# Liz490/multimodal_alzheimer

Hardware: AMD Instinct MI355X
Metric: volumes/sec fwd+bwd, 3D-ResNet-10 @128^3 bf16, 1/2/4/8 MI355X; % HBM roofline (higher is better)
Workload: dtype bf16; 1 GPU; BASELINE config 2: Anat_CNN ResNet-10 MRI-only, 1x128^3, batch 8/GPU, weighted CE, Adam, fwd+bwd+step; global_batch=8, parallelism=dp1, step_launch=hip graph replay

## Files before the change

### include/mmad.h

```cpp
#ifndef MMAD_H
#define MMAD_H

#include <stdint.h>

#ifdef __cplusplus
extern "C" {
#endif

enum { MMAD_OK = 0, MMAD_EBADSHAPE = 1001, MMAD_EBADDTYPE = 1002, MMAD_ENULL = 1003,
       MMAD_EUNSUPPORTED = 1004, MMAD_EHIP = 2000 };

enum { MMAD_F32 = 0, MMAD_BF16 = 1, MMAD_F64 = 2, MMAD_F16 = 3, MMAD_BITS = 4 };

typedef struct mmad_conv_desc {
  int32_t n;
  int32_t ci, di, hi, wi;
  int32_t co, do_, ho, wo;
  int32_t kd, kh, kw;
  int32_t sd, sh, sw;
  int32_t pd, ph, pw;
  int32_t dd, dh, dw;
} mmad_conv_desc;

int mmad_abi_version(void);
// ... 131 lines not shown
                       const void* relu_out, const void* y, const float* mean,
                       const float* invstd, float* parts, void* stream);
int mmad_bn_bwd_finalize(int c, int64_t count, int nparts, const float* parts,
                         const float* gamma, const float* invstd, int training,
                         float* dgamma, float* dbeta, float* coef, void* stream);
int mmad_bn_bwd_apply(int dtype, int64_t m, int c, const void* g, const void* g2,
                      const void* relu_out, const void* y, const float* mean,
                      const float* invstd, const float* coef, void* dy, void* gmask_out,
                      void* stream);
int mmad_bn_bwd_reduce2(int dtype, int64_t m, int c, const void* g, const void* g2,
                        int64_t g_rows, const void* relu_out, const void* y, const float* mean,
                        const float* invstd, const void* y2,
                        const float* mean2, const float* invstd2, float* parts, float* parts2,
                        void* stream);
int mmad_bn_bwd_finalize2(int c, int64_t count, int nparts, const float* parts,
                          const float* gamma, const float* invstd, int training, float* dgamma,
                          float* dbeta, float* coef, const float* parts2, const float* gamma2,
                          const float* invstd2, int training2, float* dgamma2, float* dbeta2,
                          float* coef2, void* stream);
int mmad_bn_bwd_apply2(int dtype, int64_t m, int c, const void* g, const void* g2,
                       int64_t g_rows, const void* relu_out, const void* y, const float* mean, const float* invstd, const float* coef,
                       void* dy, const void* y2, const float* mean2, const float* invstd2,
                       const float* coef2, void* dy2, void* stream);
int mmad_bn_relu_bwd_reduce(int dtype, int64_t m, int c, const void* g, const void* y,
                            const float* mean, const float* invstd, const float* scale,
                            const float* shift, float* parts, void* stream);
int mmad_bn_relu_bwd_apply(int dtype, int64_t m, int c, const void* g, const void* y,
                           const float* mean, const float* invstd, const float* scale,
                           const float* shift, const float* coef, void* dy, void* stream);
int mmad_relu_fwd(int dtype, int64_t n, const void* x, void* y, void* stream);
int mmad_relu_bwd(int dtype, int64_t n, const void* g, const void* out, void* dx, void* stream);
int mmad_add(int dtype, int64_t n, const void* a, const void* b, void* out, void* stream);

int mmad_colsum_ws(int dtype, int64_t m, int c, const void* y, float* parts, float* out,
                   void* stream);
int mmad_maxpool3d_fwd(int dtype, int n, int c, int di, int hi, int wi, int do_, int ho,
                       int wo, int k, int s, int p, const void* x, void* y,
                       uint8_t* argmax, void* stream);
int mmad_maxpool3d_bwd(int dtype, int n, int c, int di, int hi, int wi, int do_, int ho,
                       int wo, int k, int s, int p, const void* dy, const uint8_t* argmax,
                       void* dx, void* stream);
int mmad_bnpool_fwd(int dtype, int n, int c, int di, int hi, int wi, int do_, int ho, int wo,
                    int k, int s, int p, const void* y, const float* scale, const float* shift,
                    void* out, uint8_t* argmax, void* ymax, void* stream);
int mmad_bnpool_bwd_reduce(int dtype, int64_t m, int c, const void* g, const void* g2,
                           void* gsum, const uint8_t* argmax, const void* ymax,
// ... 129 lines not shown
```

### multimodal_alzheimer_amd/_lib.py

```python
import ctypes as C
import os

import torch

_PKG = os.path.dirname(os.path.abspath(__file__))
LIB_PATH = os.environ.get("MMAD_LIB_PATH") or os.path.join(_PKG, "libmmad_hip.so")

F32, BF16, F64 = 0, 1, 2
F16, BITS = 3, 4
EUNSUPPORTED = 1004
EHIP = 2000
_HIP_OOM = 2

_vp, _i32, _i64, _f32, _f64, _u64 = C.c_void_p, C.c_int, C.c_int64, C.c_float, C.c_double, C.c_uint64


class ConvDesc(C.Structure):
    _fields_ = [(n, C.c_int32) for n in (
        "n", "ci", "di", "hi", "wi", "co", "do_", "ho", "wo", "kd", "kh", "kw",
        "sd", "sh", "sw", "pd", "ph", "pw", "dd", "dh", "dw")]


class PackJob(C.Structure):
    _fields_ = ([("w", C.c_void_p), ("w_packed", C.c_void_p)] +
# ... 79 lines not shown
    "mmad_wgrad_reduce_batch": (_i32, [_i32, C.POINTER(WgradJob), _vp]),
    "mmad_stem_raw_ok": (_i32, [_P, _i32, _i32]),
    "mmad_conv3d_fwd_raw": (_i32, [_P, _i32, _vp, _i32, _vp, _vp, _vp, _vp, _vp]),
    "mmad_conv3d_wgrad_raw": (_i32, [_P, _i32, _vp, _i32, _vp, _vp, _vp, _vp, _vp, _vp]),
    "mmad_stem_dgrad_ok": (_i32, [_P, _i32, _i32]),
    "mmad_stem_dgrad_ws_bytes": (_i64, [_P]),
    "mmad_conv3d_dgrad_raw": (_i32, [_P, _i32, _vp, _vp, _i32, _vp, _vp, _vp]),
    "mmad_bn_stats_parts": (_i64, [_i64, _i32]),
    "mmad_bn_stats": (_i32, [_i32, _i64, _i32, _vp, _vp, _vp]),
    "mmad_bn_parts_fold": (_i32, [_i32, _i32, _vp, _i32, _vp, _vp]),
    "mmad_bn_finalize": (_i32, [_i32, _i64, _i32, _vp, _vp, _vp, _vp, _vp, _f32, _f32, _i32,
                                _vp, _vp, _vp, _vp, _vp, _vp]),
    "mmad_bn_finalize2": (_i32, [_i32, _i64, C.POINTER(BnFin), C.POINTER(BnFin), _vp]),
    "mmad_scale_shift_act": (_i32, [_i32, _i64, _i32, _vp, _vp, _vp, _vp, _vp, _vp, _i32, _vp,
                                    _vp]),
    "mmad_bn_bwd_parts": (_i64, [_i64, _i32]),
    "mmad_bn_bwd_reduce": (_i32, [_i32, _i64, _i32] + [_vp] * 8),
    "mmad_bn_bwd_finalize": (_i32, [_i32, _i64, _i32, _vp, _vp, _vp, _i32, _vp, _vp, _vp, _vp]),
    "mmad_bn_bwd_apply": (_i32, [_i32, _i64, _i32] + [_vp] * 10),
    "mmad_bn_bwd_reduce2": (_i32, [_i32, _i64, _i32, _vp, _vp, _i64] + [_vp] * 10),
    "mmad_bn_bwd_finalize2": (_i32, [_i32, _i64, _i32, _vp, _vp, _vp, _i32, _vp, _vp, _vp,
                                     _vp, _vp, _vp, _i32, _vp, _vp, _vp, _vp]),
    "mmad_bn_bwd_apply2": (_i32, [_i32, _i64, _i32, _vp, _vp, _i64] + [_vp] * 12),
    "mmad_relu_fwd": (_i32, [_i32, _i64, _vp, _vp, _vp]),
    "mmad_relu_bwd": (_i32, [_i32, _i64, _vp, _vp, _vp, _vp]),
    "mmad_colsum_ws": (_i32, [_i32, _i64, _i32, _vp, _vp, _vp, _vp]),
    "mmad_add": (_i32, [_i32, _i64, _vp, _vp, _vp, _vp]),
    "mmad_maxpool3d_fwd": (_i32, [_i32] * 12 + [_vp, _vp, _vp, _vp]),
    "mmad_maxpool3d_bwd": (_i32, [_i32] * 12 + [_vp, _vp, _vp, _vp]),
    "mmad_bnpool_fwd": (_i32, [_i32] * 12 + [_vp] * 7),
    "mmad_bnpool_bwd_reduce": (_i32, [_i32, _i64, _i32] + [_vp] * 9),
    "mmad_bnpool_bwd_apply": (_i32, [_i32] * 12 + [_vp] * 8),
    "mmad_gap_fwd": (_i32, [_i32, _i32, _i64, _i32, _vp, _vp, _vp]),
    "mmad_gap_fwd_ws_elems": (_i64, [_i32, _i64, _i32]),
    "mmad_conv3d_fwd_ex": (_i32, [_P, _i32, _vp, _vp, _vp, _vp, _i32, _vp, _vp, _vp]),
    "mmad_conv_pack_weight_scaled": (_i32, [_P, _i32, _vp, _vp, _vp, _i32, _vp]),
    "mmad_bn_fold": (_i32, [_i32, _vp, _vp, _vp, _vp, _f32, _vp, _vp, _vp, _vp]),
    "mmad_norm_ws_bytes": (_i64, [_i32, _i64]),
    "mmad_mri_minmax_norm": (_i32, [_i32, _i64, _vp, _vp, _f64, _vp, _vp, _vp, _vp]),
    "mmad_mri_zscore_norm": (_i32, [_i32, _i64, _vp, _vp, _vp, _vp, _vp]),
    "mmad_affine_norm": (_i32, [_i64, _vp, _f64, _f64, _vp, _vp]),
    "mmad_gap_fwd_ws": (_i32, [_i32, _i32, _i64, _i32, _vp, _vp, _vp, _vp]),
    "mmad_gap_bwd": (_i32, [_i32, _i32, _i64, _i32, _vp, _vp, _vp]),
    "mmad_gap_bwd_compact": (_i32, [_i32, _i32, _i64, _i32, _vp, _vp, _vp]),
    "mmad_gap_parts": (_i32, [_i32, _i64, _i32]),
    "mmad_gap_partial": (_i32, [_i32, _i32, _i64, _i32, _vp, _vp, _vp]),
# ... 118 lines not shown
```

### multimodal_alzheimer_amd/csrc/bn.hip

```cpp
#include "common.h"

constexpr int COLSUM_ROWS = 4;

namespace {

struct PartPlan {
  int64_t rpp;
  int nparts;
};
PartPlan part_plan(int64_t M) {
  int n = (int)std::min<int64_t>(1024, std::max<int64_t>(1, cdiv(M, 64)));
  const int64_t rpp = cdiv(M, n);
  return {rpp, (int)cdiv(M, rpp)};
}

#ifndef BN_FOLD_PROBE
#define BN_FOLD_PROBE 0
#endif
#if BN_FOLD_PROBE
__device__ int g_fold_cnt[4096];
__device__ float g_fold_sink[4096];
#endif

template <typename T, int MODE, int V, bool DUAL = false, bool G2 = false, bool GB = false>
__global__ __launch_bounds__(256) void colsum_kernel(int64_t M, int C, int64_t rpp,
                                                     const T* __restrict__ y,
                                                     const T* __restrict__ g,
                                                     const T* __restrict__ relu_out,
                                                     const float* __restrict__ mean,
                                                     const float* __restrict__ invstd,
                                                     float* __restrict__ parts,
                                                     const uint8_t* __restrict__ act,
                                                     const float* __restrict__ msc,
                                                     const float* __restrict__ msh,
                                                     const T* __restrict__ y2 = nullptr,
                                                     const float* __restrict__ mean2 = nullptr,
                                                     const float* __restrict__ invstd2 = nullptr,
                                                     float* __restrict__ parts2 = nullptr,
                                                     const T* __restrict__ g2 = nullptr,
                                                     T* __restrict__ gsum = nullptr,
                                                     uint32_t gS = 0) {
  static_assert(!DUAL || MODE == 1, "dual partial sums: BN backward with a relu_out mask");
  static_assert(!GB || (DUAL && V == Chunk<T>::N), "broadcast g: the pair kernel, 16-byte rows");
  __shared__ float red[DUAL ? 3 : 2][2048];
  const int tid = threadIdx.x;
  const int CC = C / (int)gridDim.y;
  const int cb = (int)blockIdx.y * CC;
  const int lpr = CC / V;
  const int rpar = 256 / lpr;
  const int cl = tid % lpr, rl = tid / lpr;
  const int64_t r0 = (int64_t)blockIdx.x * rpp;
  const int64_t r1 = min(M, r0 + rpp);
  float s[V], q[V], q2[V];
#pragma unroll
  for (int e = 0; e < V; ++e) { s[e] = 0.f; q[e] = 0.f; q2[e] = 0.f; }
  if (rl < rpar) {
    float mu[V], is[V], sc[V], sh[V], mu2[V], is2[V];
    if (MODE == 1 || MODE == 3 || MODE == 4) {
#pragma unroll
      for (int e = 0; e < V; ++e) { mu[e] = mean[cb + cl * V + e]; is[e] = invstd[cb + cl * V + e]; }
    }
    if constexpr (DUAL) {
#pragma unroll
      for (int e = 0; e < V; ++e) {
        mu2[e] = mean2[cb + cl * V + e];
        is2[e] = invstd2[cb + cl * V + e];
      }
    }
    if (MODE == 4) {
#pragma unroll
      for (int e = 0; e < V; ++e) { sc[e] = msc[cb + cl * V + e]; sh[e] = msh[cb + cl * V + e]; }
    }
    auto accum = [&](int64_t i, float* yv, float* gv, const float* ov, const float* y2v) {
      if (MODE == 1 || MODE == 3 || MODE == 4) {
        if (MODE == 4) {
#pragma unroll
          for (int e = 0; e < V; ++e) gv[e] = bn_affine(yv[e], sc[e], sh[e]) > 0.f ? gv[e] : 0.f;
        } else if (MODE == 3) {
#pragma unroll
          for (int e = 0; e < V; ++e) gv[e] = (act[i + e] & 0x80) ? gv[e] : 0.f;
        } else if (relu_out != nullptr) {
#pragma unroll
          for (int e = 0; e < V; ++e) gv[e] = ov[e] > 0.f ? gv[e] : 0.f;
        }
#pragma unroll
        for (int e = 0; e < V; ++e) {
          s[e] += gv[e];
          q[e] += gv[e] * ((yv[e] - mu[e]) * is[e]);
        }
        if constexpr (DUAL) {
#pragma unroll
          for (int e = 0; e < V; ++e) q2[e] += gv[e] * ((y2v[e] - mu2[e]) * is2[e]);
        }
      } else {
#pragma unroll
        for (int e = 0; e < V; ++e) {
          s[e] += yv[e];
          if (MODE == 0) q[e] += yv[e] * yv[e];
        }
      }
    };
    constexpr bool NEED_G = MODE == 1 || MODE == 3 || MODE == 4;
    int64_t r = r0 + rl;
    if constexpr (V == Chunk<T>::N) {
      constexpr int U = COLSUM_ROWS;
      for (; r + (U - 1) * rpar < r1; r += U * rpar) {
        u32x4 yr[U], gr[U], orr[U], y2r[U], g2r[U];
#pragma unroll
        for (int u = 0; u < U; ++u) {
          const int64_t i = (r + u * rpar) * C + cb + cl * V;
          yr[u] = *reinterpret_cast<const u32x4*>(y + i);
          if constexpr (GB)
            gr[u] = *reinterpret_cast<const u32x4*>(
                g + (int64_t)((uint32_t)(r + u * rpar) / gS) * C + cb + cl * V);
          else if (NEED_G)
            gr[u] = *reinterpret_cast<const u32x4*>(g + i);
          if (NEED_G && G2) g2r[u] = *reinterpret_cast<const u32x4*>(g2 + i);
          if (MODE == 1 && relu_out != nullptr)
            orr[u] = *reinterpret_cast<const u32x4*>(relu_out + i);
          if constexpr (DUAL) y2r[u] = *reinterpret_cast<const u32x4*>(y2 + i);
        }
#pragma unroll
        for (int u = 0; u < U; ++u) {
          const int64_t i = (r + u * rpar) * C + cb + cl * V;
          float yv[V], gv[V], ov[V], y2v[V];
          Chunk<T>::load(reinterpret_cast<const T*>(&yr[u]), yv);
          if (NEED_G) Chunk<T>::load(reinterpret_cast<const T*>(&gr[u]), gv);
          if constexpr (NEED_G && G2) {
            float hv[V];
            Chunk<T>::load(reinterpret_cast<const T*>(&g2r[u]), hv);
#pragma unroll
            for (int e = 0; e < V; ++e) gv[e] = as_stored<T>(gv[e] + hv[e]);
            if constexpr (MODE == 3) Chunk<T>::store(gsum + i, gv);
          }
          if (MODE == 1 && relu_out != nullptr)
            Chunk<T>::load(reinterpret_cast<const T*>(&orr[u]), ov);
          if constexpr (DUAL) Chunk<T>::load(reinterpret_cast<const T*>(&y2r[u]), y2v);
          accum(i, yv, gv, ov, y2v);
        }
      }
    }
    for (; r < r1; r += rpar) {
      const int64_t i = r * C + cb + cl * V;
      float yv[V], gv[V], ov[V], y2v[V];
      if constexpr (V == Chunk<T>::N) Chunk<T>::load(y + i, yv);
      else for (int e = 0; e < V; ++e) yv[e] = Elt<T>::ld(y, i + e);
      if (NEED_G) {
        if constexpr (GB) Chunk<T>::load(g + (int64_t)((uint32_t)r / gS) * C + cb + cl * V, gv);
        else if constexpr (V == Chunk<T>::N) Chunk<T>::load(g + i, gv);
        else for (int e = 0; e < V; ++e) gv[e] = Elt<T>::ld(g, i + e);
        if constexpr (G2) {
          float hv[V];
          if constexpr (V == Chunk<T>::N) Chunk<T>::load(g2 + i, hv);
          else for (int e = 0; e < V; ++e) hv[e] = Elt<T>::ld(g2, i + e);
#pragma unroll
          for (int e = 0; e < V; ++e) gv[e] = as_stored<T>(gv[e] + hv[e]);
          if constexpr (MODE == 3) {
            if constexpr (V == Chunk<T>::N) Chunk<T>::store(gsum + i, gv);
            else for (int e = 0; e < V; ++e) Elt<T>::st(gsum, i + e, gv[e]);
          }
        }
        if (MODE == 1 && relu_out != nullptr) {
          if constexpr (V == Chunk<T>::N) Chunk<T>::load(relu_out + i, ov);
          else for (int e = 0; e < V; ++e) ov[e] = Elt<T>::ld(relu_out, i + e);
        }
      }
      if constexpr (DUAL) {
        if constexpr (V == Chunk<T>::N) Chunk<T>::load(y2 + i, y2v);
        else for (int e = 0; e < V; ++e) y2v[e] = Elt<T>::ld(y2, i + e);
      }
      accum(i, yv, gv, ov, y2v);
    }
#pragma unroll
    for (int e = 0; e < V; ++e) {
      red[0][rl * CC + cl * V + e] = s[e];
      red[1][rl * CC + cl * V + e] = q[e];
      if constexpr (DUAL) red[DUAL ? 2 : 0][rl * CC + cl * V + e] = q2[e];
    }
  }
  __syncthreads();
  for (int c = tid; c < CC; c += 256) {
    float ss = 0.f, qq = 0.f, q2q = 0.f;
    for (int k = 0; k < rpar; ++k) {
      ss += red[0][k * CC + c];
      qq += red[1][k * CC + c];
// ... 320 lines not shown
      v[e] = relu ? fmaxf(o, 0.f) : o;
    }
  };
  int64_t q = t0;
  for (; q + stride < nchunks; q += 2 * stride) {
    float v0[N], v1[N], r0[N], r1[N];
    Chunk<T>::load(y + q * N, v0);
    Chunk<T>::load(y + (q + stride) * N, v1);
    if (RES) {
      Chunk<T>::load(res + q * N, r0);
      Chunk<T>::load(res + (q + stride) * N, r1);
    }
    apply(v0, r0);
    apply(v1, r1);
    Chunk<T>::store(out + q * N, v0);
    Chunk<T>::store(out + (q + stride) * N, v1);
  }
  if (q < nchunks) {
    float v0[N], r0[N];
    Chunk<T>::load(y + q * N, v0);
    if (RES) Chunk<T>::load(res + q * N, r0);
    apply(v0, r0);
    Chunk<T>::store(out + q * N, v0);
  }
}

template <typename T>
__global__ void scale_shift_act_scalar_kernel(int64_t M, int C, const T* __restrict__ y,
                                              const float* __restrict__ scale,
                                              const float* __restrict__ shift,
                                              const T* __restrict__ res,
                                              const float* __restrict__ rscale,
                                              const float* __restrict__ rshift, int relu,
                                              T* __restrict__ out) {
  const int64_t n = M * C;
  for (int64_t i = blockIdx.x * (int64_t)blockDim.x + threadIdx.x; i < n;
       i += (int64_t)gridDim.x * blockDim.x) {
    const int c = (int)(i % C);
    float o = bn_affine(Elt<T>::ld(y, i), scale[c], shift[c]);
    if (res) o += rscale ? Elt<T>::ld(res, i) * rscale[c] + rshift[c] : Elt<T>::ld(res, i);
    Elt<T>::st(out, i, relu ? fmaxf(o, 0.f) : o);
  }
}

struct BwdApply2 {
  const void* y2;
// ... 79 lines not shown
    Chunk<T>::load(y + (q + stride) * V, y1);
    if (relu_out) {
      Chunk<T>::load(relu_out + q * V, o0);
      Chunk<T>::load(relu_out + (q + stride) * V, o1);
    }
    if constexpr (DUAL) {
      Chunk<T>::load(y2 + q * V, z0);
      Chunk<T>::load(y2 + (q + stride) * V, z1);
    }
    one(q, g0, y0, o0, z0);
    one(q + stride, g1, y1, o1, z1);
  }
  if (q < nv) {
    float g0[V], y0[V], o0[V], z0[V];
    Chunk<T>::load(g_at(q), g0);
    if constexpr (G2) add_g2(q, g0);
    Chunk<T>::load(y + q * V, y0);
    if (relu_out) Chunk<T>::load(relu_out + q * V, o0);
    if constexpr (DUAL) Chunk<T>::load(y2 + q * V, z0);
    one(q, g0, y0, o0, z0);
  }
}

template <typename T, int V>
__global__ void bn_bwd_apply_kernel(int64_t M, int C, const T* __restrict__ g,
                                    const T* __restrict__ relu_out, const T* __restrict__ y,
                                    const float* __restrict__ mean,
                                    const float* __restrict__ invstd,
                                    const float* __restrict__ coef, T* __restrict__ dy,
                                    T* __restrict__ gmask) {
  const int64_t nv = M * C / V;
  for (int64_t q = blockIdx.x * (int64_t)blockDim.x + threadIdx.x; q < nv;
       q += (int64_t)gridDim.x * blockDim.x) {
    const int64_t i = q * V;
    const int c0 = (int)(i % C);
    float gv[V], yv[V], ov[V], dv[V];
    if constexpr (V == Chunk<T>::N) {
      Chunk<T>::load(g + i, gv);
      Chunk<T>::load(y + i, yv);
      if (relu_out) Chunk<T>::load(relu_out + i, ov);
    } else {
      for (int e = 0; e < V; ++e) {
        gv[e] = Elt<T>::ld(g, i + e);
        yv[e] = Elt<T>::ld(y, i + e);
        if (relu_out) ov[e] = Elt<T>::ld(relu_out, i + e);
      }
// ... 350 lines not shown
  const BwdApply2 d2{y2, mean2, invstd2, coef2, dy2};
  hipStream_t st = as_stream(stream);
  if (g_rows < 0 || (g_rows > 0 && (m % g_rows || m >= (int64_t(1) << 31))))
    return MMAD_EBADSHAPE;
#define APPLY2(T, G, B)                                                                      \
  hipLaunchKernelGGL((bn_bwd_apply_fc_kernel<T, false, true, G, B>), dim3(ew_grid(nv)),       \
                     dim3(256), 0, st, nv, c / vv, c, (const T*)g, (const T*)relu_out,        \
                     (const T*)y, mean, invstd, coef, (T*)dy, (T*)nullptr, nullptr, nullptr,  \
                     d2, (const T*)g2, (uint32_t)g_rows)
#define APPLY2G(T, B)                                                                        \
  do {                                                                                       \
    if (g2 != nullptr) APPLY2(T, true, B); else APPLY2(T, false, B);                         \
  } while (0)
  if (dtype == MMAD_BF16) {
    if (g_rows > 0) APPLY2G(u16, true); else APPLY2G(u16, false);
  } else {
    if (g_rows > 0) APPLY2G(float, true); else APPLY2G(float, false);
  }
#undef APPLY2G
#undef APPLY2
  return launch_status();
}

int mmad_relu_bwd(int dtype, int64_t n, const void* g, const void* out, void* dx, void* stream) {
  if (!dt_ok(dtype)) return MMAD_EBADDTYPE;
  if (n <= 0) return MMAD_EBADSHAPE;
  if (!g || !out || !dx) return MMAD_ENULL;
  if (dtype == MMAD_BF16)
    hipLaunchKernelGGL(relu_bwd_kernel<u16>, dim3(ew_grid(n)), dim3(256), 0, as_stream(stream),
                       n, (const u16*)g, (const u16*)out, (u16*)dx);
  else
    hipLaunchKernelGGL(relu_bwd_kernel<float>, dim3(ew_grid(n)), dim3(256), 0,
                       as_stream(stream), n, (const float*)g, (const float*)out, (float*)dx);
  return launch_status();
}

int mmad_relu_fwd(int dtype, int64_t n, const void* x, void* y, void* stream) {
  if (!dt_ok(dtype)) return MMAD_EBADDTYPE;
  if (n <= 0) return MMAD_EBADSHAPE;
  if (!x || !y) return MMAD_ENULL;
  if (dtype == MMAD_BF16)
    hipLaunchKernelGGL(relu_fwd_kernel<u16>, dim3(ew_grid(n)), dim3(256), 0, as_stream(stream),
                       n, (const u16*)x, (u16*)y);
  else
    hipLaunchKernelGGL(relu_fwd_kernel<float>, dim3(ew_grid(n)), dim3(256), 0,
                       as_stream(stream), n, (const float*)x, (float*)y);
// ... 18 lines not shown
```

### multimodal_alzheimer_amd/volume_ops.py

```python
import ctypes as C
import os
import weakref

import torch

from . import _lib as L

CL = torch.channels_last_3d


def _cl(t):
    if t.dim() == 5:
        return t.contiguous(memory_format=CL)
    return t.contiguous()


def _empty_vol(n, c, d, h, w, dtype, device):
    return torch.empty((n, c, d, h, w), dtype=dtype, device=device, memory_format=CL)


def _check_vol(x, dtype=None):
    L.require_device(x)
    if x.dim() != 5 or not x.is_contiguous(memory_format=CL):
        raise L.MMADError("volume tensors must be 5-D channels_last_3d (NDHWC)")
# ... 701 lines not shown
           L.stream())
    return out


def _twin_grads(g, g2, like):
    if g is None:
        g, g2 = g2, None
    out = []
    for t in (g, g2):
        if t is not None:
            t = _cl(t) if like.dim() == 5 else t.contiguous()
            if t.dtype != like.dtype:
                t = cast(t, like.dtype)
        out.append(t)
    return out


def _mask_from_y_ok(y):
    c = y.shape[1]
    v = 8 if y.dtype == torch.bfloat16 else 4
    return c % v == 0 and (c // v) & (c // v - 1) == 0 and c // v <= 256


def _bn_backward(g, relu_out, y, mean, invstd, gamma, batch_stats, want_gmask,
                 params=(None, None), mask_affine=None, g2=None, pre_parts=None):
    m, c = _rows(y)
    dev = y.device
    dt = L.dtype_code(y.dtype)
    if g2 is not None and (mask_affine is not None or not _mask_from_y_ok(y)):
        g, g2 = _sum_grads(g, g2), None
    if pre_parts is not None:
        parts = pre_parts
        nparts = parts.shape[0]
    else:
        nparts = L.load().mmad_bn_bwd_parts(m, c)
        parts = torch.empty((nparts, 2, c), dtype=torch.float32, device=dev)
    if pre_parts is not None:
        pass
    elif mask_affine is not None:
        sc, sh = mask_affine
        L.call("mmad_bn_relu_bwd_reduce", dt, m, c, L.ptr(g), L.ptr(y), L.ptr(mean),
               L.ptr(invstd), L.ptr(sc), L.ptr(sh), L.ptr(parts), L.stream())
    else:
        L.call("mmad_bn_bwd_reduce", dt, m, c, L.ptr(g), L.ptr(g2), L.ptr(relu_out), L.ptr(y),
               L.ptr(mean), L.ptr(invstd), L.ptr(parts), L.stream())
    dgamma = grad_slot(params[0], (c,), dev)
    dbeta = grad_slot(params[1], (c,), dev)
    coef = torch.empty(3 * c, dtype=torch.float32, device=dev)
    L.call("mmad_bn_bwd_finalize", c, m, nparts, L.ptr(parts), L.ptr(gamma), L.ptr(invstd),
           int(batch_stats), L.ptr(dgamma), L.ptr(dbeta), L.ptr(coef), L.stream())
    dy = torch.empty_like(y)
    gmask = torch.empty_like(y) if want_gmask else None
    if mask_affine is not None:
        L.call("mmad_bn_relu_bwd_apply", dt, m, c, L.ptr(g), L.ptr(y), L.ptr(mean),
               L.ptr(invstd), L.ptr(mask_affine[0]), L.ptr(mask_affine[1]), L.ptr(coef),
               L.ptr(dy), L.stream())
    else:
        L.call("mmad_bn_bwd_apply", dt, m, c, L.ptr(g), L.ptr(g2), L.ptr(relu_out), L.ptr(y),
               L.ptr(mean), L.ptr(invstd), L.ptr(coef), L.ptr(dy), L.ptr(gmask), L.stream())
    return dy, dgamma, dbeta, gmask


_BN_DUAL = os.environ.get("MMAD_BN_DUAL", "1") != "0"


def _bn_backward_pair(g, relu_out, y, mean, invstd, gamma, batch_stats, y2, mean2, invstd2,
                      gamma2, batch_stats2, params, params2, g2=None, g_rows=0):
    m, c = _rows(y)
    dev = y.device
    dt = L.dtype_code(y.dtype)
    nparts = L.load().mmad_bn_bwd_parts(m, c)
    parts = torch.empty((2, nparts, 2, c), dtype=torch.float32, device=dev)
    L.call("mmad_bn_bwd_reduce2", dt, m, c, L.ptr(g), L.ptr(g2), g_rows, L.ptr(relu_out),
           L.ptr(y), L.ptr(mean), L.ptr(invstd), L.ptr(y2), L.ptr(mean2), L.ptr(invstd2),
           L.ptr(parts[0]), L.ptr(parts[1]), L.stream())
    dgamma = grad_slot(params[0], (c,), dev)
    dbeta = grad_slot(params[1], (c,), dev)
    dgamma2 = grad_slot(params2[0], (c,), dev)
    dbeta2 = grad_slot(params2[1], (c,), dev)
    coef = torch.empty((2, 3 * c), dtype=torch.float32, device=dev)
    L.call("mmad_bn_bwd_finalize2", c, m, nparts, L.ptr(parts[0]), L.ptr(gamma), L.ptr(invstd),
           int(batch_stats), L.ptr(dgamma), L.ptr(dbeta), L.ptr(coef[0]), L.ptr(parts[1]),
           L.ptr(gamma2), L.ptr(invstd2), int(batch_stats2), L.ptr(dgamma2), L.ptr(dbeta2),
           L.ptr(coef[1]), L.stream())
    dy = torch.empty_like(y)
    dy2 = torch.empty_like(y2)
    L.call("mmad_bn_bwd_apply2", dt, m, c, L.ptr(g), L.ptr(g2), g_rows, L.ptr(relu_out),
           L.ptr(y), L.ptr(mean), L.ptr(invstd), L.ptr(coef[0]), L.ptr(dy), L.ptr(y2),
           L.ptr(mean2), L.ptr(invstd2), L.ptr(coef[1]), L.ptr(dy2), L.stream())
    return dy, dgamma, dbeta, dy2, dgamma2, dbeta2


class _BNActFn(torch.autograd.Function):

    @staticmethod
    def forward(ctx, y, parts, gamma, beta, res, res_parts, rgamma, rbeta, cfg):
        bn, relu, training, rbn, twin, bnsum = cfg
        L.require_device(y)
        rscale = rshift = rmean = rinvstd = None
        rbatch = False
        if rbn is not None and _BN_DUAL:
            (mean, invstd, scale, shift, batch), (rmean, rinvstd, rscale, rshift, rbatch) = \
                _finalize_pair(y, parts, bn, res, res_parts, rbn, training)
        else:
            mean, invstd, scale, shift, batch = _finalize(y, parts, bn, training)
            if rbn is not None:
                rmean, rinvstd, rscale, rshift, rbatch = _finalize(res, res_parts, rbn, training)
        out = torch.empty_like(y)
        m, c = _rows(y)
        L.call("mmad_scale_shift_act", L.dtype_code(y.dtype), m, c, L.ptr(y), L.ptr(scale),
               L.ptr(shift), L.ptr(res), L.ptr(rscale), L.ptr(rshift), int(relu), L.ptr(out),
               L.stream())
        masky = relu and res is None and y.dim() == 5 and _mask_from_y_ok(y)
        if masky and bnsum and not twin and y.dtype == torch.bfloat16:
            _BNSUM_SRC[id(out)] = (weakref.ref(out), (y, mean, invstd, scale, shift))
        ctx.save_for_backward(y, out if relu and not masky else None, mean, invstd, gamma,
                              res if rbn is not None else None, rmean, rinvstd, rgamma)
        ctx.mask_affine = (scale, shift) if masky else None
        ctx.cfg = (relu, batch, rbatch, res is not None, rbn is not None)
        ctx.params = ((gamma, beta), (rgamma, rbeta))
        if twin:
            ctx.set_materialize_grads(False)
            return out, out.view(out.shape)
        return out

    @staticmethod
    def backward(ctx, g, g2=None):
        y, out, mean, invstd, gamma, rres, rmean, rinvstd, rgamma = ctx.saved_tensors
        relu, batch, rbatch, has_res, has_rbn = ctx.cfg
        pair = (has_rbn and _BN_DUAL and out is not None and ctx.mask_affine is None
                and _mask_from_y_ok(y))
        g_rows = _gap_rows(g, y) if pair and y.numel() // y.shape[1] < 2 ** 31 else 0
        if g_rows:
            g2 = _twin_grads(g2, None, y)[0]
        else:
            g, g2 = _twin_grads(g, g2, y)
        if g is None:
            return (None,) * 9
        gam = None if gamma is None else gamma.detach()
# ... 23 lines not shown
        return (dy, None, dgamma if ctx.needs_input_grad[2] else None,
                dbeta if ctx.needs_input_grad[3] else None, dres, None,
                drg if ctx.needs_input_grad[6] else None,
                drb if ctx.needs_input_grad[7] else None, None)


def batchnorm_act(y, bn, parts=None, relu=False, res=None, res_bn=None, res_parts=None,
                  twin=False):
    if y.dim() == 5:
        _check_vol(y)
    elif not y.is_contiguous():
        raise L.MMADError("batchnorm_act expects a contiguous (B, C) tensor")
    if res is not None:
        if res.shape != y.shape or res.dtype != y.dtype:
            raise L.MMADError("residual must match the BN input in shape and dtype")
        if y.dim() == 5:
            _check_vol(res)
    training = bn.training or not bn.track_running_stats
    twin = _twin_wanted(twin, y)
    out = _BNActFn.apply(y, parts, bn.weight, bn.bias, res, res_parts,
                         None if res_bn is None else res_bn.weight,
                         None if res_bn is None else res_bn.bias,
                         (bn, relu, training, res_bn, twin,
                          BNSUM and torch.is_grad_enabled()))
    if twin:
        out, alias = out
        _register_twin(out, alias)
    return out


class _BNReluPoolFn(torch.autograd.Function):

    @staticmethod
    def forward(ctx, y, parts, gamma, beta, cfg):
        bn, training, k, s, p, twin = cfg
        mean, invstd, scale, shift, batch = _finalize(y, parts, bn, training)
        n, c, di, hi, wi = y.shape
        do, ho, wo = ((v + 2 * p - k) // s + 1 for v in (di, hi, wi))
        out = _empty_vol(n, c, do, ho, wo, y.dtype, y.device)
        ymax = torch.empty_like(out)
        am = torch.empty((n, do, ho, wo, c), dtype=torch.uint8, device=y.device)
        L.call("mmad_bnpool_fwd", L.dtype_code(y.dtype), n, c, di, hi, wi, do, ho, wo, k, s, p,
               L.ptr(y), L.ptr(scale), L.ptr(shift), L.ptr(out), L.ptr(am), L.ptr(ymax),
               L.stream())
        ctx.save_for_backward(y, am, ymax, mean, invstd, gamma)
        ctx.params = (gamma, beta)
        ctx.geo = (n, c, di, hi, wi, do, ho, wo, k, s, p)
# ... 250 lines not shown
```

Baseline: 2823 volumes/sec.

## Store residual-join ReLU masks as packed bits instead of bf16 outputs

For BN+residual+ReLU joins in training, the forward pass now writes a 1-bit-per-element ReLU mask alongside the output. The backward reduce and apply kernels read that mask, expanding bits in registers, instead of re-reading the full bf16 output tensor. This cuts the backward mask traffic from 2 bytes to 1/8 byte per element and frees the saved output for earlier release. In exchange the forward pass does an extra small byte write, and several new kernel variants and launch paths are added.

```diff
diff --git a/include/mmad.h b/include/mmad.h
--- a/include/mmad.h
+++ b/include/mmad.h
@@ -177,6 +177,26 @@
                        int64_t g_rows, const void* relu_out, const void* y, const float* mean, const float* invstd, const float* coef,
                        void* dy, const void* y2, const float* mean2, const float* invstd2,
                        const float* coef2, void* dy2, void* stream);
+int mmad_scale_shift_act_bits(int dtype, int64_t m, int c, const void* y, const float* scale,
+                              const float* shift, const void* res, const float* rscale,
+                              const float* rshift, void* out, uint8_t* relu_bits, void* stream);
+int mmad_bn_bwd_reduce_bits(int dtype, int64_t m, int c, const void* g, const void* g2,
+                            const uint8_t* relu_bits, const void* y, const float* mean,
+                            const float* invstd, float* parts, void* stream);
+int mmad_bn_bwd_apply_bits(int dtype, int64_t m, int c, const void* g, const void* g2,
+                           const uint8_t* relu_bits, const void* y, const float* mean,
+                           const float* invstd, const float* coef, void* dy, void* gmask_out,
+                           void* stream);
+int mmad_bn_bwd_reduce2_bits(int dtype, int64_t m, int c, const void* g, const void* g2,
+                             int64_t g_rows, const uint8_t* relu_bits, const void* y,
+                             const float* mean, const float* invstd, const void* y2,
+                             const float* mean2, const float* invstd2, float* parts,
+                             float* parts2, void* stream);
+int mmad_bn_bwd_apply2_bits(int dtype, int64_t m, int c, const void* g, const void* g2,
+                            int64_t g_rows, const uint8_t* relu_bits, const void* y,
+                            const float* mean, const float* invstd, const float* coef, void* dy,
+                            const void* y2, const float* mean2, const float* invstd2,
+                            const float* coef2, void* dy2, void* stream);
 int mmad_bn_relu_bwd_reduce(int dtype, int64_t m, int c, const void* g, const void* y,
                             const float* mean, const float* invstd, const float* scale,
                             const float* shift, float* parts, void* stream);
diff --git a/multimodal_alzheimer_amd/_lib.py b/multimodal_alzheimer_amd/_lib.py
--- a/multimodal_alzheimer_amd/_lib.py
+++ b/multimodal_alzheimer_amd/_lib.py
@@ -125,6 +125,11 @@
     "mmad_bn_bwd_finalize2": (_i32, [_i32, _i64, _i32, _vp, _vp, _vp, _i32, _vp, _vp, _vp,
                                      _vp, _vp, _vp, _i32, _vp, _vp, _vp, _vp]),
     "mmad_bn_bwd_apply2": (_i32, [_i32, _i64, _i32, _vp, _vp, _i64] + [_vp] * 12),
+    "mmad_scale_shift_act_bits": (_i32, [_i32, _i64, _i32] + [_vp] * 9),
+    "mmad_bn_bwd_reduce_bits": (_i32, [_i32, _i64, _i32] + [_vp] * 8),
+    "mmad_bn_bwd_apply_bits": (_i32, [_i32, _i64, _i32] + [_vp] * 10),
+    "mmad_bn_bwd_reduce2_bits": (_i32, [_i32, _i64, _i32, _vp, _vp, _i64] + [_vp] * 10),
+    "mmad_bn_bwd_apply2_bits": (_i32, [_i32, _i64, _i32, _vp, _vp, _i64] + [_vp] * 12),
     "mmad_relu_fwd": (_i32, [_i32, _i64, _vp, _vp, _vp]),
     "mmad_relu_bwd": (_i32, [_i32, _i64, _vp, _vp, _vp, _vp]),
     "mmad_colsum_ws": (_i32, [_i32, _i64, _i32, _vp, _vp, _vp, _vp]),
diff --git a/multimodal_alzheimer_amd/csrc/bn.hip b/multimodal_alzheimer_amd/csrc/bn.hip
--- a/multimodal_alzheimer_amd/csrc/bn.hip
+++ b/multimodal_alzheimer_amd/csrc/bn.hip
@@ -40,7 +40,9 @@
                                                      const T* __restrict__ g2 = nullptr,
                                                      T* __restrict__ gsum = nullptr,
                                                      uint32_t gS = 0) {
-  static_assert(!DUAL || MODE == 1, "dual partial sums: BN backward with a relu_out mask");
+  static_assert(!DUAL || MODE == 1 || MODE == 5,
+                "dual partial sums: BN backward with a relu_out mask");
+  static_assert(MODE != 5 || (sizeof(T) == 2 && V == 8), "bit masks: bf16 channel vectors");
   static_assert(!GB || (DUAL && V == Chunk<T>::N), "broadcast g: the pair kernel, 16-byte rows");
   __shared__ float red[DUAL ? 3 : 2][2048];
   const int tid = threadIdx.x;
@@ -56,7 +58,7 @@
   for (int e = 0; e < V; ++e) { s[e] = 0.f; q[e] = 0.f; q2[e] = 0.f; }
   if (rl < rpar) {
     float mu[V], is[V], sc[V], sh[V], mu2[V], is2[V];
-    if (MODE == 1 || MODE == 3 || MODE == 4) {
+    if (MODE == 1 || MODE == 3 || MODE == 4 || MODE == 5) {
 #pragma unroll
       for (int e = 0; e < V; ++e) { mu[e] = mean[cb + cl * V + e]; is[e] = invstd[cb + cl * V + e]; }
     }
@@ -72,7 +74,7 @@
       for (int e = 0; e < V; ++e) { sc[e] = msc[cb + cl * V + e]; sh[e] = msh[cb + cl * V + e]; }
     }
     auto accum = [&](int64_t i, float* yv, float* gv, const float* ov, const float* y2v) {
-      if (MODE == 1 || MODE == 3 || MODE == 4) {
+      if (MODE == 1 || MODE == 3 || MODE == 4 || MODE == 5) {
         if (MODE == 4) {
 #pragma unroll
           for (int e = 0; e < V; ++e) gv[e] = bn_affine(yv[e], sc[e], sh[e]) > 0.f ? gv[e] : 0.f;
@@ -100,12 +102,18 @@
         }
       }
     };
-    constexpr bool NEED_G = MODE == 1 || MODE == 3 || MODE == 4;
+    constexpr bool NEED_G = MODE == 1 || MODE == 3 || MODE == 4 || MODE == 5;
+    const uint8_t* __restrict__ relu_bits = reinterpret_cast<const uint8_t*>(relu_out);
+    auto expand = [](uint32_t mb, float* ov) {
+#pragma unroll
+      for (int e = 0; e < V; ++e) ov[e] = ((mb >> e) & 1u) ? 1.f : 0.f;
+    };
     int64_t r = r0 + rl;
     if constexpr (V == Chunk<T>::N) {
       constexpr int U = COLSUM_ROWS;
       for (; r + (U - 1) * rpar < r1; r += U * rpar) {
         u32x4 yr[U], gr[U], orr[U], y2r[U], g2r[U];
+        uint32_t mr[U];
 #pragma unroll
         for (int u = 0; u < U; ++u) {
           const int64_t i = (r + u * rpar) * C + cb + cl * V;
@@ -116,7 +124,9 @@
           else if (NEED_G)
             gr[u] = *reinterpret_cast<const u32x4*>(g + i);
           if (NEED_G && G2) g2r[u] = *reinterpret_cast<const u32x4*>(g2 + i);
-          if (MODE == 1 && relu_out != nullptr)
+          if constexpr (MODE == 5)
+            mr[u] = relu_bits[i >> 3];
+          else if (MODE == 1 && relu_out != nullptr)
             orr[u] = *reinterpret_cast<const u32x4*>(relu_out + i);
           if constexpr (DUAL) y2r[u] = *reinterpret_cast<const u32x4*>(y2 + i);
         }
@@ -133,7 +143,9 @@
             for (int e = 0; e < V; ++e) gv[e] = as_stored<T>(gv[e] + hv[e]);
             if constexpr (MODE == 3) Chunk<T>::store(gsum + i, gv);
           }
-          if (MODE == 1 && relu_out != nullptr)
+          if constexpr (MODE == 5)
+            expand(mr[u], ov);
+          else if (MODE == 1 && relu_out != nullptr)
             Chunk<T>::load(reinterpret_cast<const T*>(&orr[u]), ov);
           if constexpr (DUAL) Chunk<T>::load(reinterpret_cast<const T*>(&y2r[u]), y2v);
           accum(i, yv, gv, ov, y2v);
@@ -160,7 +172,9 @@
             else for (int e = 0; e < V; ++e) Elt<T>::st(gsum, i + e, gv[e]);
           }
         }
-        if (MODE == 1 && relu_out != nullptr) {
+        if constexpr (MODE == 5) {
+          expand(relu_bits[i >> 3], ov);
+        } else if (MODE == 1 && relu_out != nullptr) {
           if constexpr (V == Chunk<T>::N) Chunk<T>::load(relu_out + i, ov);
           else for (int e = 0; e < V; ++e) ov[e] = Elt<T>::ld(relu_out, i + e);
         }
@@ -527,6 +541,61 @@
     if (RES) Chunk<T>::load(res + q * N, r0);
     apply(v0, r0);
     Chunk<T>::store(out + q * N, v0);
+  }
+}
+
+template <int RES>
+__global__ __launch_bounds__(256) void scale_shift_act_bits_kernel(
+    int64_t nchunks, int cpr, const u16* __restrict__ y, const float* __restrict__ scale,
+    const float* __restrict__ shift, const u16* __restrict__ res,
+    const float* __restrict__ rscale, const float* __restrict__ rshift, u16* __restrict__ out,
+    uint8_t* __restrict__ bits) {
+  static_assert(RES == 1 || RES == 2, "residual joins only");
+  constexpr int N = 8;
+  const int64_t t0 = (int64_t)blockIdx.x * 256 + threadIdx.x;
+  const int64_t stride = (int64_t)gridDim.x * 256;
+  const int c0 = (int)(t0 & (cpr - 1)) * N;
+  float sc[N], sh[N], rs[N], rh[N];
+  ld_params<N>(scale + c0, sc);
+  ld_params<N>(shift + c0, sh);
+  if (RES == 2) {
+    ld_params<N>(rscale + c0, rs);
+    ld_params<N>(rshift + c0, rh);
+  }
+  auto apply_store = [&](int64_t q, float* v, const float* r) {
+#pragma unroll
+    for (int e = 0; e < N; ++e) {
+      float o = bn_affine(v[e], sc[e], sh[e]);
+      if (RES == 1) o += r[e];
+      if (RES == 2) o += r[e] * rs[e] + rh[e];
+      v[e] = fmaxf(o, 0.f);
+    }
+    u32x4 c;
+    uint32_t mb = 0;
+#pragma unroll
+    for (int i = 0; i < 4; ++i) {
+      c[i] = pack_bf16x2(v[2 * i], v[2 * i + 1]);
+      mb |= (bf2f((u16)(c[i] & 0xffffu)) > 0.f ? 1u : 0u) << (2 * i);
+      mb |= (bf2f((u16)(c[i] >> 16)) > 0.f ? 1u : 0u) << (2 * i + 1);
+    }
+    *reinterpret_cast<u32x4*>(out + q * N) = c;
+    bits[q] = (uint8_t)mb;
+  };
+  int64_t q = t0;
+  for (; q + stride < nchunks; q += 2 * stride) {
+    float v0[N], v1[N], r0[N], r1[N];
+    Chunk<u16>::load(y + q * N, v0);
+    Chunk<u16>::load(y + (q + stride) * N, v1);
+    Chunk<u16>::load(res + q * N, r0);
+    Chunk<u16>::load(res + (q + stride) * N, r1);
+    apply_store(q, v0, r0);
+    apply_store(q + stride, v1, r1);
+  }
+  if (q < nchunks) {
+    float v0[N], r0[N];
+    Chunk<u16>::load(y + q * N, v0);
+    Chunk<u16>::load(res + q * N, r0);
+    apply_store(q, v0, r0);
   }
 }
 
@@ -652,6 +721,92 @@
   }
 }
 
+template <bool DUAL, bool G2, bool GB>
+__global__ __launch_bounds__(256) void bn_bwd_apply_bits_kernel(
+    int64_t nv, int cpr, int C, const u16* __restrict__ g, const uint8_t* __restrict__ relu_bits,
+    const u16* __restrict__ y, const float* __restrict__ mean, const float* __restrict__ invstd,
+    const float* __restrict__ coef, u16* __restrict__ dy, u16* __restrict__ gmask, BwdApply2 d2,
+    const u16* __restrict__ g2, uint32_t gS) {
+  using T = u16;
+  constexpr int V = 8;
+  const int cpr_shift = __builtin_ctz(cpr);
+  auto g_at = [&](int64_t qq) -> const T* {
+    if constexpr (GB)
+      return g + (int64_t)((uint32_t)(qq >> cpr_shift) / gS) * C + (qq & (cpr - 1)) * V;
+    else
+      return g + qq * V;
+  };
+  const int64_t t0 = (int64_t)blockIdx.x * 256 + threadIdx.x;
+  const int64_t stride = (int64_t)gridDim.x * 256;
+  const int c0 = (int)(t0 & (cpr - 1)) * V;
+  float mu[V], is[V], k0[V], k1[V], k2[V];
+  ld_params<V>(mean + c0, mu);
+  ld_params<V>(invstd + c0, is);
+  ld_params<V>(coef + c0, k0);
+  ld_params<V>(coef + C + c0, k1);
+  ld_params<V>(coef + 2 * C + c0, k2);
+  const T* __restrict__ y2 = static_cast<const T*>(d2.y2);
+  T* __restrict__ dy2 = static_cast<T*>(d2.dy2);
+  float mu2[V], is2[V], j0[V], j1[V], j2[V];
+  if constexpr (DUAL) {
+    ld_params<V>(d2.mean2 + c0, mu2);
+    ld_params<V>(d2.invstd2 + c0, is2);
+    ld_params<V>(d2.coef2 + c0, j0);
+    ld_params<V>(d2.coef2 + C + c0, j1);
+    ld_params<V>(d2.coef2 + 2 * C + c0, j2);
+  }
+  auto one = [&](int64_t q, const float* gv0, const float* yv, uint32_t mb, const float* y2v) {
+    float gv[V], dv[V], dv2[V];
+#pragma unroll
+    for (int e = 0; e < V; ++e) {
+      gv[e] = ((mb >> e) & 1u) ? gv0[e] : 0.f;
+      const float xh = (yv[e] - mu[e]) * is[e];
+      dv[e] = k0[e] * gv[e] - k1[e] - xh * k2[e];
+      if constexpr (DUAL) {
+        const float xh2 = (y2v[e] - mu2[e]) * is2[e];
+        dv2[e] = j0[e] * gv[e] - j1[e] - xh2 * j2[e];
+      }
+    }
+    Chunk<T>::store(dy + q * V, dv);
+    if constexpr (DUAL) Chunk<T>::store(dy2 + q * V, dv2);
+    if (gmask) Chunk<T>::store(gmask + q * V, gv);
+  };
+  auto add_g2 = [&](int64_t qq, float* gv) {
+    float hv[V];
+    Chunk<T>::load(g2 + qq * V, hv);
+#pragma unroll
+    for (int e = 0; e < V; ++e) gv[e] = as_stored<T>(gv[e] + hv[e]);
+  };
+  int64_t q = t0;
+  for (; q + stride < nv; q += 2 * stride) {
+    float g0[V], g1[V], y0[V], y1[V], z0[V], z1[V];
+    Chunk<T>::load(g_at(q), g0);
+    Chunk<T>::load(g_at(q + stride), g1);
+    if constexpr (G2) {
+      add_g2(q, g0);
+      add_g2(q + stride, g1);
+    }
+    Chunk<T>::load(y + q * V, y0);
+    Chunk<T>::load(y + (q + stride) * V, y1);
+    const uint32_t m0 = relu_bits[q], m1 = relu_bits[q + stride];
+    if constexpr (DUAL) {
+      Chunk<T>::load(y2 + q * V, z0);
+      Chunk<T>::load(y2 + (q + stride) * V, z1);
+    }
+    one(q, g0, y0, m0, z0);
+    one(q + stride, g1, y1, m1, z1);
+  }
+  if (q < nv) {
+    float g0[V], y0[V], z0[V];
+    Chunk<T>::load(g_at(q), g0);
+    if constexpr (G2) add_g2(q, g0);
+    Chunk<T>::load(y + q * V, y0);
+    const uint32_t m0 = relu_bits[q];
+    if constexpr (DUAL) Chunk<T>::load(y2 + q * V, z0);
+    one(q, g0, y0, m0, z0);
+  }
+}
+
 template <typename T, int V>
 __global__ void bn_bwd_apply_kernel(int64_t M, int C, const T* __restrict__ g,
                                     const T* __restrict__ relu_out, const T* __restrict__ y,
@@ -1048,6 +1203,124 @@
   return launch_status();
 }
 
+static bool bits_layout_ok(int dtype, int c) {
+  return dtype == MMAD_BF16 && c % 8 == 0 && is_pow2(c / 8) && c / 8 <= 256;
+}
+
+int mmad_scale_shift_act_bits(int dtype, int64_t m, int c, const void* y, const float* scale,
+                              const float* shift, const void* res, const float* rscale,
+                              const float* rshift, void* out, uint8_t* relu_bits, void* stream) {
+  if (!dt_ok(dtype)) return MMAD_EBADDTYPE;
+  if (m <= 0 || c <= 0) return MMAD_EBADSHAPE;
+  if (!y || !scale || !shift || !res || !out || !relu_bits) return MMAD_ENULL;
+  if ((rscale == nullptr) != (rshift == nullptr)) return MMAD_ENULL;
+  if (!bits_layout_ok(dtype, c)) return MMAD_EUNSUPPORTED;
+  const int64_t nv = m * c / 8;
+#define SSAB(R)                                                                              \
+  hipLaunchKernelGGL((scale_shift_act_bits_kernel<R>), dim3(ew_grid(nv)), dim3(256), 0,       \
+                     as_stream(stream), nv, c / 8, (const u16*)y, scale, shift,                \
+                     (const u16*)res, rscale, rshift, (u16*)out, relu_bits)
+  if (rscale == nullptr) SSAB(1); else SSAB(2);
+#undef SSAB
+  return launch_status();
+}
+
+static int launch_colsum_bits(int64_t m, int c, const void* g, const void* g2, int64_t g_rows,
+                              const uint8_t* relu_bits, const void* y, const float* mean,
+                              const float* invstd, const void* y2, const float* mean2,
+                              const float* invstd2, float* parts, float* parts2,
+                              hipStream_t st) {
+  const PartPlan pp = part_plan(m);
+  const bool h = g2 != nullptr;
+  auto k = y2 == nullptr ? (h ? colsum_kernel<u16, 5, 8, false, true> : colsum_kernel<u16, 5, 8>)
+           : g_rows > 0  ? (h ? colsum_kernel<u16, 5, 8, true, true, true>
+                              : colsum_kernel<u16, 5, 8, true, false, true>)
+                         : (h ? colsum_kernel<u16, 5, 8, true, true>
+                              : colsum_kernel<u16, 5, 8, true, false>);
+  hipLaunchKernelGGL(k, dim3((unsigned)pp.nparts), dim3(256), 0, st, m, c, pp.rpp, (const u16*)y,
+                     (const u16*)g, reinterpret_cast<const u16*>(relu_bits), mean, invstd, parts,
+                     (const uint8_t*)nullptr, (const float*)nullptr, (const float*)nullptr,
+                     (const u16*)y2, mean2, invstd2, parts2, (const u16*)g2, (u16*)nullptr,
+                     (uint32_t)g_rows);
+  return launch_status();
+}
+
+static int launch_apply_bits(int64_t m, int c, const void* g, const void* g2, int64_t g_rows,
+                             const uint8_t* relu_bits, const void* y, const float* mean,
+                             const float* invstd, const float* coef, void* dy, void* gmask,
+                             const BwdApply2* d2, hipStream_t st) {
+  const int64_t nv = m * c / 8;
+  const bool h = g2 != nullptr;
+  auto k = d2 == nullptr ? (h ? bn_bwd_apply_bits_kernel<false, true, false>
+                              : bn_bwd_apply_bits_kernel<false, false, false>)
+           : g_rows > 0  ? (h ? bn_bwd_apply_bits_kernel<true, true, true>
+                              : bn_bwd_apply_bits_kernel<true, false, true>)
+                         : (h ? bn_bwd_apply_bits_kernel<true, true, false>
+                              : bn_bwd_apply_bits_kernel<true, false, false>);
+  hipLaunchKernelGGL(k, dim3(ew_grid(nv)), dim3(256), 0, st, nv, c / 8, c, (const u16*)g,
+                     relu_bits, (const u16*)y, mean, invstd, coef, (u16*)dy, (u16*)gmask,
+                     d2 ? *d2 : BwdApply2{}, (const u16*)g2, (uint32_t)g_rows);
+  return launch_status();
+}
+
+int mmad_bn_bwd_reduce_bits(int dtype, int64_t m, int c, const void* g, const void* g2,
+                            const uint8_t* relu_bits, const void* y, const float* mean,
+                            const float* invstd, float* parts, void* stream) {
+  if (!dt_ok(dtype)) return MMAD_EBADDTYPE;
+  if (m <= 0 || c <= 0) return MMAD_EBADSHAPE;
+  if (!g || !relu_bits || !y || !mean || !invstd || !parts) return MMAD_ENULL;
+  if (!bits_layout_ok(dtype, c)) return MMAD_EUNSUPPORTED;
+  return launch_colsum_bits(m, c, g, g2, 0, relu_bits, y, mean, invstd, nullptr, nullptr,
+                            nullptr, parts, nullptr, as_stream(stream));
+}
+
+int mmad_bn_bwd_apply_bits(int dtype, int64_t m, int c, const void* g, const void* g2,
+                           const uint8_t* relu_bits, const void* y, const float* mean,
+                           const float* invstd, const float* coef, void* dy, void* gmask,
+                           void* stream) {
+  if (!dt_ok(dtype)) return MMAD_EBADDTYPE;
+  if (m <= 0 || c <= 0) return MMAD_EBADSHAPE;
+  if (!g || !relu_bits || !y || !mean || !invstd || !coef || !dy) return MMAD_ENULL;
+  if (!bits_layout_ok(dtype, c)) return MMAD_EUNSUPPORTED;
+  return launch_apply_bits(m, c, g, g2, 0, relu_bits, y, mean, invstd, coef, dy, gmask, nullptr,
+                           as_stream(stream));
+}
+
+int mmad_bn_bwd_reduce2_bits(int dtype, int64_t m, int c, const void* g, const void* g2,
+                             int64_t g_rows, const uint8_t* relu_bits, const void* y,
+                             const float* mean, const float* invstd, const void* y2,
+                             const float* mean2, const float* invstd2, float* parts,
+                             float* parts2, void* stream) {
+  if (!dt_ok(dtype)) return MMAD_EBADDTYPE;
+  if (m <= 0 || c <= 0) return MMAD_EBADSHAPE;
+  if (!g || !relu_bits || !y || !mean || !invstd || !y2 || !mean2 || !invstd2 || !parts ||
+      !parts2)
+    return MMAD_ENULL;
+  if (g_rows < 0 || (g_rows > 0 && (m % g_rows || m >= (int64_t(1) << 31))))
+    return MMAD_EBADSHAPE;
+  if (!bits_layout_ok(dtype, c)) return MMAD_EUNSUPPORTED;
+  return launch_colsum_bits(m, c, g, g2, g_rows, relu_bits, y, mean, invstd, y2, mean2, invstd2,
+                            parts, parts2, as_stream(stream));
+}
+
+int mmad_bn_bwd_apply2_bits(int dtype, int64_t m, int c, const void* g, const void* g2,
+                            int64_t g_rows, const uint8_t* relu_bits, const void* y,
+                            const float* mean, const float* invstd, const float* coef, void* dy,
+                            const void* y2, const float* mean2, const float* invstd2,
+                            const float* coef2, void* dy2, void* stream) {
+  if (!dt_ok(dtype)) return MMAD_EBADDTYPE;
+  if (m <= 0 || c <= 0) return MMAD_EBADSHAPE;
+  if (!g || !relu_bits || !y || !mean || !invstd || !coef || !dy || !y2 || !mean2 || !invstd2 ||
+      !coef2 || !dy2)
+    return MMAD_ENULL;
+  if (g_rows < 0 || (g_rows > 0 && (m % g_rows || m >= (int64_t(1) << 31))))
+    return MMAD_EBADSHAPE;
+  if (!bits_layout_ok(dtype, c)) return MMAD_EUNSUPPORTED;
+  const BwdApply2 d2{y2, mean2, invstd2, coef2, dy2};
+  return launch_apply_bits(m, c, g, g2, g_rows, relu_bits, y, mean, invstd, coef, dy, nullptr,
+                           &d2, as_stream(stream));
+}
+
 int mmad_relu_bwd(int dtype, int64_t n, const void* g, const void* out, void* dx, void* stream) {
   if (!dt_ok(dtype)) return MMAD_EBADDTYPE;
   if (n <= 0) return MMAD_EBADSHAPE;
diff --git a/multimodal_alzheimer_amd/volume_ops.py b/multimodal_alzheimer_amd/volume_ops.py
--- a/multimodal_alzheimer_amd/volume_ops.py
+++ b/multimodal_alzheimer_amd/volume_ops.py
@@ -747,11 +747,24 @@
     return c % v == 0 and (c // v) & (c // v - 1) == 0 and c // v <= 256
 
 
+RELU_BITS = os.environ.get("MMAD_RELU_BITS", "1") != "0"
+
+
+def _relu_bits_wanted(y, res, relu, training):
+    return (RELU_BITS and relu and res is not None and training and torch.is_grad_enabled()
+            and y.dim() == 5 and y.dtype == torch.bfloat16 and _mask_from_y_ok(y))
+
+
+def _is_bits(mask):
+    return mask is not None and mask.dtype == torch.uint8
+
+
 def _bn_backward(g, relu_out, y, mean, invstd, gamma, batch_stats, want_gmask,
                  params=(None, None), mask_affine=None, g2=None, pre_parts=None):
     m, c = _rows(y)
     dev = y.device
     dt = L.dtype_code(y.dtype)
+    sfx = "_bits" if _is_bits(relu_out) else ""
     if g2 is not None and (mask_affine is not None or not _mask_from_y_ok(y)):
         g, g2 = _sum_grads(g, g2), None
     if pre_parts is not None:
@@ -767,8 +780,8 @@
         L.call("mmad_bn_relu_bwd_reduce", dt, m, c, L.ptr(g), L.ptr(y), L.ptr(mean),
                L.ptr(invstd), L.ptr(sc), L.ptr(sh), L.ptr(parts), L.stream())
     else:
-        L.call("mmad_bn_bwd_reduce", dt, m, c, L.ptr(g), L.ptr(g2), L.ptr(relu_out), L.ptr(y),
-               L.ptr(mean), L.ptr(invstd), L.ptr(parts), L.stream())
+        L.call("mmad_bn_bwd_reduce" + sfx, dt, m, c, L.ptr(g), L.ptr(g2), L.ptr(relu_out),
+               L.ptr(y), L.ptr(mean), L.ptr(invstd), L.ptr(parts), L.stream())
     dgamma = grad_slot(params[0], (c,), dev)
     dbeta = grad_slot(params[1], (c,), dev)
     coef = torch.empty(3 * c, dtype=torch.float32, device=dev)
@@ -781,8 +794,9 @@
                L.ptr(invstd), L.ptr(mask_affine[0]), L.ptr(mask_affine[1]), L.ptr(coef),
                L.ptr(dy), L.stream())
     else:
-        L.call("mmad_bn_bwd_apply", dt, m, c, L.ptr(g), L.ptr(g2), L.ptr(relu_out), L.ptr(y),
-               L.ptr(mean), L.ptr(invstd), L.ptr(coef), L.ptr(dy), L.ptr(gmask), L.stream())
+        L.call("mmad_bn_bwd_apply" + sfx, dt, m, c, L.ptr(g), L.ptr(g2), L.ptr(relu_out),
+               L.ptr(y), L.ptr(mean), L.ptr(invstd), L.ptr(coef), L.ptr(dy), L.ptr(gmask),
+               L.stream())
     return dy, dgamma, dbeta, gmask
 
 
@@ -794,9 +808,10 @@
     m, c = _rows(y)
     dev = y.device
     dt = L.dtype_code(y.dtype)
+    sfx = "_bits" if _is_bits(relu_out) else ""
     nparts = L.load().mmad_bn_bwd_parts(m, c)
     parts = torch.empty((2, nparts, 2, c), dtype=torch.float32, device=dev)
-    L.call("mmad_bn_bwd_reduce2", dt, m, c, L.ptr(g), L.ptr(g2), g_rows, L.ptr(relu_out),
+    L.call("mmad_bn_bwd_reduce2" + sfx, dt, m, c, L.ptr(g), L.ptr(g2), g_rows, L.ptr(relu_out),
            L.ptr(y), L.ptr(mean), L.ptr(invstd), L.ptr(y2), L.ptr(mean2), L.ptr(invstd2),
            L.ptr(parts[0]), L.ptr(parts[1]), L.stream())
     dgamma = grad_slot(params[0], (c,), dev)
@@ -810,7 +825,7 @@
            L.ptr(coef[1]), L.stream())
     dy = torch.empty_like(y)
     dy2 = torch.empty_like(y2)
-    L.call("mmad_bn_bwd_apply2", dt, m, c, L.ptr(g), L.ptr(g2), g_rows, L.ptr(relu_out),
+    L.call("mmad_bn_bwd_apply2" + sfx, dt, m, c, L.ptr(g), L.ptr(g2), g_rows, L.ptr(relu_out),
            L.ptr(y), L.ptr(mean), L.ptr(invstd), L.ptr(coef[0]), L.ptr(dy), L.ptr(y2),
            L.ptr(mean2), L.ptr(invstd2), L.ptr(coef[1]), L.ptr(dy2), L.stream())
     return dy, dgamma, dbeta, dy2, dgamma2, dbeta2
@@ -820,7 +835,7 @@
 
     @staticmethod
     def forward(ctx, y, parts, gamma, beta, res, res_parts, rgamma, rbeta, cfg):
-        bn, relu, training, rbn, twin, bnsum = cfg
+        bn, relu, training, rbn, twin, bnsum, bits = cfg
         L.require_device(y)
         rscale = rshift = rmean = rinvstd = None
         rbatch = False
@@ -833,13 +848,22 @@
                 rmean, rinvstd, rscale, rshift, rbatch = _finalize(res, res_parts, rbn, training)
         out = torch.empty_like(y)
         m, c = _rows(y)
-        L.call("mmad_scale_shift_act", L.dtype_code(y.dtype), m, c, L.ptr(y), L.ptr(scale),
-               L.ptr(shift), L.ptr(res), L.ptr(rscale), L.ptr(rshift), int(relu), L.ptr(out),
-               L.stream())
+        mask = None
+        if bits:
+            mask = torch.empty((m, c // 8), dtype=torch.uint8, device=y.device)
+            L.call("mmad_scale_shift_act_bits", L.dtype_code(y.dtype), m, c, L.ptr(y),
+                   L.ptr(scale), L.ptr(shift), L.ptr(res), L.ptr(rscale), L.ptr(rshift),
+                   L.ptr(out), L.ptr(mask), L.stream())
+        else:
+            L.call("mmad_scale_shift_act", L.dtype_code(y.dtype), m, c, L.ptr(y), L.ptr(scale),
+                   L.ptr(shift), L.ptr(res), L.ptr(rscale), L.ptr(rshift), int(relu),
+                   L.ptr(out), L.stream())
         masky = relu and res is None and y.dim() == 5 and _mask_from_y_ok(y)
         if masky and bnsum and not twin and y.dtype == torch.bfloat16:
             _BNSUM_SRC[id(out)] = (weakref.ref(out), (y, mean, invstd, scale, shift))
-        ctx.save_for_backward(y, out if relu and not masky else None, mean, invstd, gamma,
+        if mask is None and relu and not masky:
+            mask = out
+        ctx.save_for_backward(y, mask, mean, invstd, gamma,
                               res if rbn is not None else None, rmean, rinvstd, rgamma)
         ctx.mask_affine = (scale, shift) if masky else None
         ctx.cfg = (relu, batch, rbatch, res is not None, rbn is not None)
@@ -909,7 +933,8 @@
                          None if res_bn is None else res_bn.weight,
                          None if res_bn is None else res_bn.bias,
                          (bn, relu, training, res_bn, twin,
-                          BNSUM and torch.is_grad_enabled()))
+                          BNSUM and torch.is_grad_enabled(),
+                          _relu_bits_wanted(y, res, relu, training)))
     if twin:
         out, alias = out
         _register_twin(out, alias)
```

After: 2836 volumes/sec (median of 6 runs). No clear change (+0.5%).
